# hangg7/soar

Hardware: AMD Instinct MI355X
Metric: fwd+bwd frames/sec @100k Gaussians, 1080p; achieved HBM GB/s vs roofline (higher is better)
Workload: dtype f32

## Files before the change

### include/soar_hip.h

```cpp
#ifndef SOAR_HIP_H
#define SOAR_HIP_H

#include <stddef.h>
#include <stdint.h>

#ifdef __cplusplus
extern "C" {
#endif

#define SOAR_HIP_ABI_VERSION 8

typedef struct SoarRastParams {
    int32_t P;
    int32_t W, H;
    int32_t sh_degree;
    int32_t M;
    int32_t prefiltered;
    int32_t render_front;
    int32_t sort_descending;
    int32_t debug;
    int32_t cfg_surface;
    int32_t cfg_normalize_depth;
    int32_t cfg_perpix_depth;
    int32_t cfg_lrn_cam;
// ... 234 lines not shown
                             SoarLossFinish *finish_out, void *stream);
int soar_frame_loss_pooled_partials(int32_t W, int32_t H, const float *color, const float *normal, const float *depth,
                                    const float *opac, const float *target_pool, int32_t n_sets, const int32_t *set_index_dev,
                                    float w_color, float w_mask, float w_normal, float w_depth, float *loss_out, float *scratch,
                                    float *dL_dcolor, float *dL_dnormal, float *dL_ddepth, float *dL_dopac, const void *image_buffer,
                                    const float *background, int32_t normalize_depth, SoarLossFinish *finish_out, void *stream);

#define SOAR_BACKWARD_LOSS_SCRATCH_FLOATS (4 * SOAR_FRAME_LOSS_SCRATCH_FLOATS)
typedef struct SoarBackwardLoss {
    const float *color, *normal, *depth, *opac;
    const float *target_color, *target_mask, *target_normal;
    const int32_t *set_index_dev;
    int32_t n_sets;
    float w_color, w_mask, w_normal, w_depth;
    float *loss_out;
    float *wave_sums;
} SoarBackwardLoss;
int soar_rast_backward_plan_loss(const SoarRastParams *prm, int32_t region,
                                 const float *means3D, const int32_t *radii, const float *shs,
                                 const float *colors_precomp, const float *scales, const float *rotations,
                                 const float *cov3D_precomp,
                                 const void *geom_buffer, const void *binning_buffer, const void *image_buffer,
                                 int64_t num_rendered, const SoarBackwardLoss *loss,
                                 float *dL_dmeans2D, float *dL_dcolors, float *dL_dopacity, float *dL_dmeans3D,
                                 float *dL_dcov3D, float *dL_dsh, float *dL_dscales, float *dL_drotations,
                                 float *dL_dviewmat, float *dL_dprojmat, float *dL_dcampos,
                                 void *workspace, size_t workspace_bytes, SoarLossFinish *finish_out,
                                 void *stream);
int soar_frames_geometry_warp_backward_wave_losses(int32_t n, const SoarFrameTail *frames, const float *xyz, const float *rot,
                                                   const float *weights, const float *joint_mats, int32_t P, int32_t J, const float *scales,
                                                   float *dL_dxyz, float *dL_drot, float *dL_dscales, float *dL_dcolors, float *dL_docc,
                                                   const SoarLossFinish *finish, void *stream);

typedef struct SoarAvatarLossArgs {
    int32_t H, W;
    float cos_limit, cos_weight;
    const float *render, *gt_rgb;
    const float *mask_img, *gt_mask;
    const float *normal, *gt_normal;
    const float *occ;
    const uint8_t *sel, *sel_normal, *sel_occ;
    float *stats, *stats_occ;
    float *scratch;
    const float *counts;
    const float *up_l1, *up_l1m, *up_cos, *up_occ, *up_ssim;
    const float *g_ssim;
    float *g_render, *g_mask, *g_normal, *g_occ;
    int32_t normal_raw;
    int32_t occ_grad_summed;
    float *cos_scale_out;
    const float *background;
} SoarAvatarLossArgs;
int soar_avatar_loss_scratch_floats(size_t *count);
int soar_avatar_pixel_losses(const SoarAvatarLossArgs *args, int32_t mode, void *stream);

int soar_ssim_scratch_floats(int32_t C, int32_t H, int32_t W, size_t *count);
int soar_ssim(int32_t C, int32_t H, int32_t W, const float *img1, const float *img2, float *ssim_out, float *scratch,
              float *dssim_dimg1, void *stream);
int soar_ssim_rendered(int32_t C, int32_t H, int32_t W, const float *img1, const float *img2, float *ssim_out, float *scratch,
                       float *dssim_dimg1, const float *rendered, void *stream);

typedef struct SoarDensifyRow {
    const float *src;
    float *dst;
    int32_t width;
    int32_t mode;
// ... 526 lines not shown
```

### soar_amd/csrc/lbs.hip

```cpp
#include "soar_common.h"
#include "loss_finish.h"
#include "geom_bwd_point.h"
#include "preprocess_point.h"
#include "soar_quat.h"

#pragma clang fp contract(on)

#ifndef SOAR_LBS_SKIP_UNUSED_JOINTS
#define SOAR_LBS_SKIP_UNUSED_JOINTS 1
#endif

namespace soar {

namespace {

constexpr int KNN_TILE = 1024;

__device__ __forceinline__ void quat_to_mat(const float q[4], float m[9])
{
    const float r = q[0], i = q[1], j = q[2], k = q[3];
    const float two_s = 2.0f / (r * r + i * i + j * j + k * k);
    m[0] = 1 - two_s * (j * j + k * k); m[1] = two_s * (i * j - k * r); m[2] = two_s * (i * k + j * r);
    m[3] = two_s * (i * j + k * r); m[4] = 1 - two_s * (i * i + k * k); m[5] = two_s * (j * k - i * r);
    m[6] = two_s * (i * k - j * r); m[7] = two_s * (j * k + i * r); m[8] = 1 - two_s * (i * i + j * j);
// ... 328 lines not shown
    }
#pragma unroll
    for (int h = 0; h < 2; h++) {
        const int o = tid + h * WARP_THREADS, c = o / WAVE, q = p0 + o % WAVE;
        if (o < 7 * WAVE && q < a.P) {
            if (c < 3) a.g_xyz[3 * q + c] = acc[h];
            else a.g_rot[4 * q + c - 3] = acc[h];
        }
    }
    if (p < a.P && k >= 1 && k - 1 < fs.n_extra) {
        const int e = k - 1, w = fs.width[e];
        const size_t count = (size_t)a.P * w;
        const float *src = fs.src[e] + (size_t)p * w;
        float *dst = fs.dst[e] + (size_t)p * w;
        for (int c0 = 0; c0 < w; c0 += 4) {
            float v[4][WARP_NF];
#pragma unroll
            for (int c = 0; c < 4; c++)
#pragma unroll
                for (int f = 0; f < WARP_NF; f++) v[c][f] = (c0 + c < w && f < n) ? src[(size_t)f * count + c0 + c] : 0.f;
#pragma unroll
            for (int c = 0; c < 4; c++) {
                if (c0 + c >= w) break;
                float s = v[c][0];
#pragma unroll
                for (int f = 1; f < WARP_NF; f++) s = f < n ? s + v[c][f] : s;
                for (int f = WARP_NF; f < n; f++) s += src[(size_t)f * count + c0 + c];
                dst[c0 + c] = s;
            }
        }
    }
}

__global__ void __launch_bounds__(WARP_THREADS) warp_preprocess_frames_kernel(WarpArgs a, int n, Batch<PreArgs> fr)
{
    extern __shared__ float wtile[];
    const int tid = threadIdx.x, k = __builtin_amdgcn_readfirstlane(tid / WAVE), lane = tid % WAVE;
    const int p0 = blockIdx.x * WAVE, p_raw = p0 + lane;
    stage_weight_rows(a, wtile, tid, p0);
    const int f = blockIdx.y * WARP_NF + k;
    if (f >= n) return;
    const bool in_range = p_raw < a.P;
    const int p = in_range ? p_raw : a.P - 1;
    float M[12], pos[3];
    float4 quat;
    blend_frame_matrix(wtile + (p - p0) * a.J, a.joint_mats + (size_t)f * a.mats_stride, a.J, M);
    forward_point_vals(a, p, M, pos, quat);
    float *xyz_out = a.xyz_out + (size_t)f * a.xyz_stride, *rot_out = a.rot_out + (size_t)f * a.rot_stride;
    xyz_out[3 * p] = pos[0]; xyz_out[3 * p + 1] = pos[1]; xyz_out[3 * p + 2] = pos[2];
    reinterpret_cast<float4 *>(rot_out)[p] = quat;
    const PreArgs &g = fr.v[f];
    PrePoint o;
    preprocess_point(g, p, in_range, pos[0], pos[1], pos[2], true, quat, o);
    preprocess_store(g, p, in_range, blockIdx.x, o);
    if (!g.prefiltered && blockIdx.x == 0 && lane == 0) g.header[H_PREFILTER_VIOLATIONS] = 0u;
}

constexpr int TAIL_C = 14;
struct TailOut {
    float *dL_dmeans2D[MAX_BATCH];
    float *dL_dscales, *dL_dcolors, *dL_docc;
};
struct TailLosses {
    int n, first_block;
    int per_wave;
    SoarLossFinish v[MAX_BATCH];
};
#ifndef SOAR_TAIL_WPE
#define SOAR_TAIL_WPE 4
#endif
__global__ void __launch_bounds__(WARP_THREADS) __attribute__((amdgpu_waves_per_eu(SOAR_TAIL_WPE, 8))) geom_warp_backward_frames_kernel(WarpArgs a, int n, Batch<GeomBwdArgs> fr, TailOut out, TailLosses losses)
{
    extern __shared__ __attribute__((aligned(16))) float wtile[];
    static_assert(WARP_THREADS == 256 && WARP_NF * TAIL_C * WAVE * sizeof(float) >= 256 * sizeof(float4), "loss_finish_sum: 256 threads, 4 KB of LDS");
    if (losses.n && (int)blockIdx.x >= losses.first_block) {
        const SoarLossFinish &l = losses.v[(int)blockIdx.x - losses.first_block];
        if (losses.per_wave) loss_finish_sum<true>(l.sums4, l.blocks, l.n, l.w_color, l.w_mask, l.w_normal, l.w_depth, l.loss_out, reinterpret_cast<float4 *>(wtile));
        else loss_finish_sum(l.sums4, l.blocks, l.n, l.w_color, l.w_mask, l.w_normal, l.w_depth, l.loss_out, reinterpret_cast<float4 *>(wtile));
        return;
    }
    float *red = wtile + WAVE * a.J;
    const int tid = threadIdx.x, k = __builtin_amdgcn_readfirstlane(tid / WAVE), lane = tid % WAVE;
    const int p0 = blockIdx.x * WAVE, p = p0 + lane;
    stage_weight_rows(a, wtile, tid, p0);
    constexpr int PER = (TAIL_C * WAVE + WARP_THREADS - 1) / WARP_THREADS;
    float acc[PER];
#pragma unroll
    for (int h = 0; h < PER; h++) acc[h] = 0.f;
    for (int f0 = 0; f0 < n; f0 += WARP_NF) {
        const int f = f0 + k;
        float d[TAIL_C];
#pragma unroll
        for (int c = 0; c < TAIL_C; c++) d[c] = 0.f;
        if (p < a.P && f < n) {
            const GeomBwdArgs &g = fr.v[f];
            GeomBwdPoint o;
            geometry_backward_point<false>(g, p, g.radii[p] > 0, o, nullptr, nullptr, nullptr);
            float *m2 = out.dL_dmeans2D[f];
            m2[3 * p + 0] = o.acc[0]; m2[3 * p + 1] = o.acc[1]; m2[3 * p + 2] = 0.f;
            float M[12], dx[3];
            float4 dq;
            blend_frame_matrix(wtile + lane * a.J, a.joint_mats + (size_t)f * a.mats_stride, a.J, M);
            backward_point_vals(a, p, M, o.g_mean[0], o.g_mean[1], o.g_mean[2], make_float4(o.g_rot[0], o.g_rot[1], o.g_rot[2], o.g_rot[3]), dx, dq);
            d[0] = dx[0]; d[1] = dx[1]; d[2] = dx[2]; d[3] = dq.x; d[4] = dq.y; d[5] = dq.z; d[6] = dq.w;
            d[7] = o.g_scale[0]; d[8] = o.g_scale[1]; d[9] = o.g_scale[2];
            d[10] = o.acc[6]; d[11] = o.acc[7]; d[12] = o.acc[8];
            d[13] = o.acc[13];
        }
        if (f0) __syncthreads();
#pragma unroll
        for (int c = 0; c < TAIL_C; c++) red[(k * TAIL_C + c) * WAVE + lane] = d[c];
        __syncthreads();
#pragma unroll
        for (int h = 0; h < PER; h++) {
            const int o = tid + h * WARP_THREADS;
            if (o < TAIL_C * WAVE)
#pragma unroll
                for (int kk = 0; kk < WARP_NF; kk++) acc[h] += red[kk * TAIL_C * WAVE + o];
        }
    }
#pragma unroll
    for (int h = 0; h < PER; h++) {
        const int o = tid + h * WARP_THREADS, c = o / WAVE, q = p0 + o % WAVE;
        if (o < TAIL_C * WAVE && q < a.P) {
            if (c < 3) a.g_xyz[3 * q + c] = acc[h];
            else if (c < 7) a.g_rot[4 * q + c - 3] = acc[h];
            else if (c < 10) out.dL_dscales[3 * q + c - 7] = acc[h];
            else if (c < 13) out.dL_dcolors[3 * q + c - 10] = acc[h];
            else if (out.dL_docc) out.dL_docc[q] = acc[h];
        }
    }
}

__global__ void __launch_bounds__(256) dist2_knn3_kernel(const float *__restrict__ pts, int N, float *__restrict__ out)
{
    __shared__ float tile[KNN_TILE * 3];
    const int tid = threadIdx.x;
    const int p = blockIdx.x * 256 + tid;
    const bool valid = p < N;
    float x = 0.f, y = 0.f, z = 0.f;
    if (valid) { x = pts[3 * p]; y = pts[3 * p + 1]; z = pts[3 * p + 2]; }
    float b0 = 3.402823466e+38f, b1 = b0, b2 = b0;
    for (int base = 0; base < N; base += KNN_TILE) {
        const int n = min(KNN_TILE, N - base);
        __syncthreads();
        for (int t = tid; t < n * 3; t += 256) tile[t] = pts[(size_t)base * 3 + t];
        __syncthreads();
        if (!valid) continue;
        for (int v = 0; v < n; v++) {
            const float ddx = x - tile[3 * v], ddy = y - tile[3 * v + 1], ddz = z - tile[3 * v + 2];
            float d = ddx * ddx + ddy * ddy + ddz * ddz;
            if (base + v == p) continue;
            if (d < b2) {
                b2 = d;
                if (b2 < b1) { const float t = b1; b1 = b2; b2 = t; }
                if (b1 < b0) { const float t = b0; b0 = b1; b1 = t; }
            }
        }
    }
    if (valid) out[p] = (b0 + b1 + b2) / 3.0f;
}

}

// ... 90 lines not shown

static int warp_backward_frames(const float *xyz, const float *rot, const float *weights, const float *joint_mats, const float *axis_perm,
                                size_t mats_stride, int32_t n, int32_t P, int32_t J, const float *dL_dxyz_out, const float *dL_drot_out,
                                float *dL_dxyz, float *dL_drot, int32_t n_extra, const float *const *extra_src, float *const *extra_dst,
                                const int32_t *extra_width, void *stream_)
{
    hipStream_t stream = static_cast<hipStream_t>(stream_);
    if (n <= 0 || !weights) { set_error("soar_lbs_warp_backward_sum: need n > 0 and blend weights"); return 1; }
    if (n_extra < 0 || n_extra > 2 || (n_extra > 0 && (!extra_src || !extra_dst || !extra_width))) {
        set_error("soar_lbs_warp_backward_sum: at most two extra blocks");
        return 1;
    }
    if (warp_check(xyz, rot, weights, joint_mats, P, J)) return 1;
    if (P == 0) return 0;
    if (!dL_dxyz_out || !dL_drot_out || !dL_dxyz || !dL_drot) { set_error("soar_lbs_warp_backward_sum: NULL pointer"); return 1; }
    WarpArgs a{};
    a.P = P; a.J = J; a.xyz = xyz; a.rot = rot; a.weights = weights; a.joint_mats = joint_mats;
    a.g_xyz_out = dL_dxyz_out; a.g_rot_out = dL_drot_out; a.g_xyz = dL_dxyz; a.g_rot = dL_drot;
    a.axis_perm = axis_perm;
    a.mats_stride = mats_stride; a.xyz_stride = (size_t)P * 3; a.rot_stride = (size_t)P * 4;
    FrameSums fs{};
    fs.n_extra = n_extra;
    for (int e = 0; e < n_extra; e++) {
        if (!extra_src[e] || !extra_dst[e] || extra_width[e] <= 0) { set_error("soar_lbs_warp_backward_sum: bad extra block %d", e); return 1; }
        fs.src[e] = extra_src[e]; fs.dst[e] = extra_dst[e]; fs.width[e] = extra_width[e];
    }
    const size_t lds = sizeof(float) * (WAVE * (size_t)J + WARP_NF * 7 * WAVE);
    StageTimer timer(ST_LBS_WARP_BWD, stream);
    hipLaunchKernelGGL(warp_backward_frames_kernel, dim3((P + WAVE - 1) / WAVE), dim3(WARP_THREADS), lds, stream, a, (int)n, fs);
    SOAR_LAUNCH_OK("lbs_warp_backward_sum", stream, 0);
    return 0;
}

int soar_frames_warp_preprocess(int32_t n, const SoarFrameHead *frames, const float *xyz, const float *rot, const float *weights,
                                const float *joint_mats, int32_t P, int32_t J, const float *colors, const float *opacities, const float *scales,
                                float *xyz_out, float *rot_out, void *stream_)
{
    hipStream_t stream = static_cast<hipStream_t>(stream_);
    const char *who = "soar_frames_warp_preprocess";
    if (n < 1 || n > MAX_BATCH || !frames) { set_error("%s: 1 <= n <= %d frames", who, MAX_BATCH); return 1; }
    if (!weights) { set_error("%s: needs the blend weights", who); return 1; }
    if (warp_check(xyz, rot, weights, joint_mats, P, J)) return 1;
    if (P == 0) return 0;
    if (!colors || !opacities || !scales || !xyz_out || !rot_out) { set_error("%s: a required pointer is NULL", who); return 1; }
    WarpArgs a{};
    a.P = P; a.J = J; a.xyz = xyz; a.rot = rot; a.weights = weights; a.joint_mats = joint_mats;
    a.xyz_out = xyz_out; a.rot_out = rot_out;
    a.mats_stride = (size_t)J * 16; a.xyz_stride = (size_t)P * 3; a.rot_stride = (size_t)P * 4;
    Batch<PreArgs> fr{};
    for (int f = 0; f < n; f++) {
        const SoarFrameHead &t = frames[f];
        if (!t.prm || !t.geom_buffer || !t.radii) { set_error("%s: frame %d: a pointer is NULL", who, f); return 1; }
        if (t.prm->P != P || t.prm->M != 0 || t.prm->prefiltered != 0) {
            set_error("%s: frame %d: needs P = %d Gaussians with explicit colours (M = 0), not prefiltered", who, f, P);
            return 1;
        }
        GeomBuf g;
        carve_geom(t.geom_buffer, P, 0, &g);
        fill_pre_args(fr.v[f], *t.prm, xyz_out + (size_t)f * a.xyz_stride, nullptr, colors, opacities, scales, rot_out + (size_t)f * a.rot_stride,
                      nullptr, g, t.radii);
    }
    const size_t lds = sizeof(float) * WAVE * (size_t)J;
    StageTimer timer(ST_LBS_WARP_FWD, stream);
    hipLaunchKernelGGL(warp_preprocess_frames_kernel, dim3((P + WAVE - 1) / WAVE, (n + WARP_NF - 1) / WARP_NF), dim3(WARP_THREADS), lds, stream,
                       a, (int)n, fr);
    SOAR_LAUNCH_OK("frames_warp_preprocess", stream, 0);
    return 0;
}

int soar_frames_geometry_warp_backward(int32_t n, const SoarFrameTail *frames, const float *xyz, const float *rot, const float *weights,
                                       const float *joint_mats, int32_t P, int32_t J, const float *scales, float *dL_dxyz, float *dL_drot,
                                       float *dL_dscales, float *dL_dcolors, float *dL_docc, void *stream_)
{
    return soar_frames_geometry_warp_backward_losses(n, frames, xyz, rot, weights, joint_mats, P, J, scales, dL_dxyz, dL_drot, dL_dscales,
                                                     dL_dcolors, dL_docc, nullptr, stream_);
}

static int frames_tail(int32_t n, const SoarFrameTail *frames, const float *xyz, const float *rot, const float *weights, const float *joint_mats,
                       int32_t P, int32_t J, const float *scales, float *dL_dxyz, float *dL_drot, float *dL_dscales, float *dL_dcolors,
                       float *dL_docc, const SoarLossFinish *finish, bool per_wave, const char *who, void *stream_);

int soar_frames_geometry_warp_backward_losses(int32_t n, const SoarFrameTail *frames, const float *xyz, const float *rot,
                                              const float *weights, const float *joint_mats, int32_t P, int32_t J, const float *scales,
                                              float *dL_dxyz, float *dL_drot, float *dL_dscales, float *dL_dcolors, float *dL_docc,
                                              const SoarLossFinish *finish, void *stream_)
{
    return frames_tail(n, frames, xyz, rot, weights, joint_mats, P, J, scales, dL_dxyz, dL_drot, dL_dscales, dL_dcolors, dL_docc, finish, false,
                       finish ? "soar_frames_geometry_warp_backward_losses" : "soar_frames_geometry_warp_backward", stream_);
}

int soar_frames_geometry_warp_backward_wave_losses(int32_t n, const SoarFrameTail *frames, const float *xyz, const float *rot,
                                                   const float *weights, const float *joint_mats, int32_t P, int32_t J, const float *scales,
                                                   float *dL_dxyz, float *dL_drot, float *dL_dscales, float *dL_dcolors, float *dL_docc,
                                                   const SoarLossFinish *finish, void *stream_)
{
    if (!finish) { set_error("soar_frames_geometry_warp_backward_wave_losses: finish is NULL"); return 1; }
    return frames_tail(n, frames, xyz, rot, weights, joint_mats, P, J, scales, dL_dxyz, dL_drot, dL_dscales, dL_dcolors, dL_docc, finish, true,
                       "soar_frames_geometry_warp_backward_wave_losses", stream_);
}

static int frames_tail(int32_t n, const SoarFrameTail *frames, const float *xyz, const float *rot, const float *weights, const float *joint_mats,
                       int32_t P, int32_t J, const float *scales, float *dL_dxyz, float *dL_drot, float *dL_dscales, float *dL_dcolors,
                       float *dL_docc, const SoarLossFinish *finish, bool per_wave, const char *who, void *stream_)
{
    hipStream_t stream = static_cast<hipStream_t>(stream_);
    if (n < 1 || n > MAX_BATCH || !frames) { set_error("%s: 1 <= n <= %d frames", who, MAX_BATCH); return 1; }
    if (!weights) { set_error("%s: needs the blend weights", who); return 1; }
    if (warp_check(xyz, rot, weights, joint_mats, P, J)) return 1;
    if (P == 0) return 0;
    if (!scales || !dL_dxyz || !dL_drot || !dL_dscales || !dL_dcolors) { set_error("%s: a required pointer is NULL", who); return 1; }
    WarpArgs a{};
    a.P = P; a.J = J; a.xyz = xyz; a.rot = rot; a.weights = weights; a.joint_mats = joint_mats;
    a.g_xyz = dL_dxyz; a.g_rot = dL_drot;
    a.mats_stride = (size_t)J * 16;
    Batch<GeomBwdArgs> fr{};
    TailOut out{};
    out.dL_dscales = dL_dscales; out.dL_dcolors = dL_dcolors; out.dL_docc = dL_docc;
    for (int f = 0; f < n; f++) {
        const SoarFrameTail &t = frames[f];
        if (!t.prm || !t.means3D || !t.rotations || !t.radii || !t.geom_buffer || !t.workspace || !t.dL_dmeans2D) {
            set_error("%s: frame %d: a pointer is NULL", who, f);
            return 1;
        }
        if (t.prm->P != P || t.prm->M != 0 || t.prm->cfg_lrn_cam != 0) {
            set_error("%s: frame %d: needs P = %d Gaussians with explicit colours (M = 0) and cfg_lrn_cam = 0", who, f, P);
            return 1;
        }
        GeomBuf g;
        carve_geom(const_cast<void *>(t.geom_buffer), P, 0, &g);
        fill_geom_bwd_args(fr.v[f], *t.prm, t.means3D, t.radii, nullptr, scales, t.rotations, nullptr, g, static_cast<const float *>(t.workspace));
        out.dL_dmeans2D[f] = t.dL_dmeans2D;
    }
    TailLosses losses{};
    const int blocks = (P + WAVE - 1) / WAVE;
    if (finish) {
        losses.n = n; losses.first_block = blocks; losses.per_wave = per_wave ? 1 : 0;
        for (int f = 0; f < n; f++) {
            const SoarLossFinish &l = finish[f];
            if (!l.sums4 || !l.loss_out || l.blocks < 1 || l.blocks > SOAR_FRAME_LOSS_SCRATCH_FLOATS / 4 || l.n < 1) {
                set_error("%s: frame %d: finish[] is not what %s left", who, f,
                          per_wave ? "soar_rast_backward_plan_loss" : "soar_frame_loss_partials");
                return 1;
            }
            losses.v[f] = l;
        }
    }
    const size_t lds = sizeof(float) * (WAVE * (size_t)J + WARP_NF * TAIL_C * WAVE);
    StageTimer timer(ST_LBS_WARP_BWD, stream);
    hipLaunchKernelGGL(geom_warp_backward_frames_kernel, dim3(blocks + losses.n), dim3(WARP_THREADS), lds, stream, a, (int)n, fr, out, losses);
    SOAR_LAUNCH_OK("frames_geometry_warp_backward", stream, 0);
    return 0;
}

int soar_dist2_knn3(const float *points, int32_t N, float *out, void *stream_)
{
    hipStream_t stream = static_cast<hipStream_t>(stream_);
    if (N < 0) { set_error("soar_dist2_knn3: N < 0"); return 1; }
    if (N == 0) return 0;
    if (!points || !out) { set_error("soar_dist2_knn3: NULL pointer"); return 1; }
    StageTimer timer(ST_DIST2, stream);
    hipLaunchKernelGGL(dist2_knn3_kernel, dim3((N + 255) / 256), dim3(256), 0, stream, points, N, out);
    SOAR_LAUNCH_OK("dist2_knn3", stream, 0);
    return 0;
}

}
```

### soar_amd/hip_lib.py

```python
from __future__ import annotations

import ctypes as C
import os
from typing import Optional

_HERE = os.path.dirname(os.path.abspath(__file__))
LIB_PATH = os.environ.get("SOAR_HIP_LIB") or os.path.join(_HERE, "_lib", "libsoar_hip.so")
if os.environ.get("SOAR_HIP_LIB"):
    import sys as _sys
    print(f"[soar_amd] SOAR_HIP_LIB is set: loading {LIB_PATH} instead of the in-tree build (development A/B runs only)", file=_sys.stderr)

FRAME_LOSS_SCRATCH_FLOATS = 4 * 2048
ABI_VERSION = 8
c_f32p = C.c_void_p
_vp = C.c_void_p


class SoarRastParams(C.Structure):
    _fields_ = [
        ("P", C.c_int32), ("W", C.c_int32), ("H", C.c_int32), ("sh_degree", C.c_int32), ("M", C.c_int32),
        ("prefiltered", C.c_int32), ("render_front", C.c_int32), ("sort_descending", C.c_int32), ("debug", C.c_int32),
        ("cfg_surface", C.c_int32), ("cfg_normalize_depth", C.c_int32), ("cfg_perpix_depth", C.c_int32),
        ("cfg_lrn_cam", C.c_int32),
        ("tanfovx", C.c_float), ("tanfovy", C.c_float), ("scale_modifier", C.c_float),
# ... 223 lines not shown
    "soar_rast_backward_plan": (C.c_int, [C.POINTER(SoarRastParams), C.c_int32] + [_vp] * 7 + [_vp, _vp, _vp, C.c_int64] + [_vp] * 4
                                + [_vp] * 11 + [_vp, C.c_size_t, _vp]),
    "soar_rast_backward_plan_loss": (C.c_int, [C.POINTER(SoarRastParams), C.c_int32] + [_vp] * 7 + [_vp, _vp, _vp, C.c_int64] + [_vp]
                                     + [_vp] * 11 + [_vp, C.c_size_t, _vp, _vp]),
    "soar_rast_backward_occ_plan": (C.c_int, [C.POINTER(SoarRastParams), C.c_int32] + [_vp] * 7 + [_vp, _vp, _vp, C.c_int64] + [_vp] * 6
                                    + [C.c_int32] + [_vp] * 12 + [_vp, C.c_size_t, _vp]),
    "soar_rast_backward_region_counts": (C.c_int, [C.POINTER(C.c_int64), C.POINTER(C.c_int64)]),
    "soar_batch_begin": (C.c_int, [C.c_int32]),
    "soar_batch_frame": (C.c_int, [C.c_int32]),
    "soar_batch_end": (C.c_int, []),
    "soar_rast_occ_backward": (C.c_int, [C.POINTER(SoarRastParams), _vp, _vp, _vp, C.c_int64, _vp, _vp, _vp]),
    "soar_rast_mark_visible": (C.c_int, [C.c_int32, _vp, _vp, _vp, _vp, _vp]),
    "soar_rast_export_state": (C.c_int, [C.POINTER(SoarRastParams), _vp, _vp, _vp, C.c_int64] + [_vp] * 17 + [_vp]),
    "soar_lbs_knn_weights_bytes": (C.c_int, [C.c_int32, C.c_int32, C.POINTER(C.c_size_t)]),
    "soar_lbs_knn_weights": (C.c_int, [_vp, C.c_int32, _vp, C.c_int32, _vp, C.c_int32, C.c_int32, _vp, _vp, _vp, C.c_size_t, _vp]),
    "soar_lbs_knn_grid_bytes": (C.c_int, [C.c_int32, C.POINTER(C.c_size_t)]),
    "soar_lbs_knn_query_bytes": (C.c_int, [C.c_int32, C.POINTER(C.c_size_t)]),
    "soar_lbs_knn_build_grid": (C.c_int, [_vp, C.c_int32, _vp, C.c_int32, _vp, _vp]),
    "soar_lbs_knn_query": (C.c_int, [_vp, C.c_int32, _vp, C.c_int32, _vp, C.c_int32, C.c_int32, _vp, _vp, _vp, C.c_size_t, _vp]),
    "soar_lbs_knn_query_ordered": (C.c_int, [_vp, C.c_int32, _vp, C.c_int32, _vp, C.c_int32, C.c_int32, _vp, C.c_int32, _vp, _vp,
                                             _vp, C.c_size_t, _vp]),
    "soar_lbs_knn_state_bytes": (C.c_int, [C.c_int32, C.POINTER(C.c_size_t)]),
    "soar_lbs_knn_query_state": (C.c_int, [_vp, C.c_int32, _vp, C.c_int32, _vp, C.c_int32, _vp, C.c_int32, _vp, _vp, _vp, C.c_size_t, _vp]),
    "soar_lbs_knn_refresh": (C.c_int, [_vp, C.c_int32, C.c_int32, _vp, C.c_int32, _vp, _vp, _vp, _vp, _vp]),
    "soar_lbs_warp_forward": (C.c_int, [_vp] * 6 + [C.c_int32, C.c_int32] + [_vp] * 4),
    "soar_lbs_warp_backward": (C.c_int, [_vp] * 5 + [C.c_int32, C.c_int32] + [_vp] * 5),
    "soar_lbs_warp_forward_batch": (C.c_int, [_vp] * 4 + [C.c_int32] * 3 + [_vp] * 3),
    "soar_lbs_warp_backward_sum": (C.c_int, [_vp] * 4 + [C.c_int32] * 3 + [_vp] * 4 + [C.c_int32, _vp, _vp, _vp, _vp]),
    "soar_frames_warp_preprocess": (C.c_int, [C.c_int32, _vp] + [_vp] * 4 + [C.c_int32, C.c_int32] + [_vp] * 6),
    "soar_rast_backward_rows": (C.c_int, [_vp] * 22),
    "soar_frames_geometry_warp_backward": (C.c_int, [C.c_int32, _vp] + [_vp] * 4 + [C.c_int32, C.c_int32] + [_vp] * 7),
    "soar_frames_geometry_warp_backward_losses": (C.c_int, [C.c_int32, _vp] + [_vp] * 4 + [C.c_int32, C.c_int32] + [_vp] * 8),
    "soar_frames_geometry_warp_backward_wave_losses": (C.c_int, [C.c_int32, _vp] + [_vp] * 4 + [C.c_int32, C.c_int32] + [_vp] * 8),
    "soar_dist2_knn3": (C.c_int, [_vp, C.c_int32, _vp, _vp]),
    "soar_depth2normal": (C.c_int, [C.c_int32, C.c_int32, _vp, _vp, C.c_float, C.c_float, C.c_float, C.c_float, _vp, _vp]),
    "soar_depth2normal_backward": (C.c_int, [C.c_int32, C.c_int32, _vp, _vp, C.c_float, C.c_float, C.c_float, C.c_float, _vp, _vp,
                                             _vp]),
    "soar_normal2curv": (C.c_int, [C.c_int32, C.c_int32, _vp, _vp, _vp, _vp]),
    "soar_normal2curv_backward": (C.c_int, [C.c_int32, C.c_int32, _vp, _vp, _vp, _vp, _vp]),
    "soar_view_finish": (C.c_int, [C.c_int32, C.c_int32, _vp, _vp, _vp, _vp, C.c_float, C.c_float, _vp, _vp, _vp, _vp]),
    "soar_view_finish_backward": (C.c_int, [C.c_int32, C.c_int32, _vp, _vp, _vp, _vp, C.c_float, C.c_float, _vp, _vp, _vp, _vp,
                                            _vp, _vp]),
    "soar_ssim_scratch_floats": (C.c_int, [C.c_int32, C.c_int32, C.c_int32, C.POINTER(C.c_size_t)]),
    "soar_ssim": (C.c_int, [C.c_int32, C.c_int32, C.c_int32, _vp, _vp, _vp, _vp, _vp, _vp]),
    "soar_ssim_rendered": (C.c_int, [C.c_int32, C.c_int32, C.c_int32, _vp, _vp, _vp, _vp, _vp, _vp, _vp]),
    "soar_densify_stats": (C.c_int, [C.c_int32, _vp, _vp, C.c_int32, _vp, _vp, _vp, _vp, _vp, _vp]),
    "soar_densify_plan_bytes": (C.c_int, [C.c_int32, C.POINTER(C.c_size_t)]),
    "soar_densify_plan": (C.c_int, [C.c_int32, _vp, _vp, _vp, C.c_int32, C.c_int32, C.c_float, C.c_float, C.c_float, C.c_float,
                                    C.c_float, _vp, C.POINTER(C.c_int64), _vp]),
    "soar_densify_flags": (C.c_int, [C.c_int32, _vp, _vp, _vp]),
    "soar_densify_apply": (C.c_int, [C.c_int32, C.c_int32, _vp, C.c_int32, C.POINTER(SoarDensifyRow), _vp, _vp, _vp, C.c_int32, _vp]),
    "soar_smplx_joint_mats": (C.c_int, [C.c_int32, C.c_int32, C.c_int32, _vp, C.c_int32, _vp, _vp, _vp, _vp, _vp, _vp, _vp, _vp]),
    "soar_image_loss_scratch_floats": (C.c_int, [C.POINTER(C.c_size_t)]),
    "soar_masked_l1": (C.c_int, [C.c_int32, C.c_int32, C.c_int32, _vp, _vp, _vp, _vp, _vp, _vp]),
    "soar_masked_l1_backward": (C.c_int, [C.c_int32, C.c_int32, C.c_int32, _vp, _vp, _vp, _vp, _vp, _vp, _vp]),
    "soar_cos_loss": (C.c_int, [C.c_int32, C.c_int32, C.c_int32, _vp, _vp, _vp, C.c_float, C.c_float, _vp, _vp, _vp]),
    "soar_cos_loss_backward": (C.c_int, [C.c_int32, C.c_int32, C.c_int32, _vp, _vp, _vp, C.c_float, C.c_float, _vp, _vp, _vp, _vp]),
    "soar_frame_loss": (C.c_int, [C.c_int32, C.c_int32, _vp, _vp, _vp, _vp, _vp, _vp, _vp, C.c_float, C.c_float, C.c_float,
                                  C.c_float, _vp, _vp, _vp, _vp, _vp, _vp, _vp, _vp, C.c_int32, _vp]),
    "soar_frame_loss_pooled": (C.c_int, [C.c_int32, C.c_int32, _vp, _vp, _vp, _vp, _vp, C.c_int32, _vp, C.c_float, C.c_float, C.c_float,
                                         C.c_float, _vp, _vp, _vp, _vp, _vp, _vp, _vp, _vp, C.c_int32, _vp]),
    "soar_frame_loss_partials": (C.c_int, [C.c_int32, C.c_int32, _vp, _vp, _vp, _vp, _vp, _vp, _vp, C.c_float, C.c_float, C.c_float,
                                           C.c_float, _vp, _vp, _vp, _vp, _vp, _vp, _vp, _vp, C.c_int32, _vp, _vp]),
    "soar_frame_loss_pooled_partials": (C.c_int, [C.c_int32, C.c_int32, _vp, _vp, _vp, _vp, _vp, C.c_int32, _vp, C.c_float, C.c_float,
                                                  C.c_float, C.c_float, _vp, _vp, _vp, _vp, _vp, _vp, _vp, _vp, C.c_int32, _vp, _vp]),
    "soar_selftest_exp": (C.c_int, [_vp, C.c_int32, _vp, _vp, _vp]),
# ... 165 lines not shown
```

### soar_amd/step_plan.py

```python
from __future__ import annotations

import ctypes as C
import os
from typing import Dict, List, Optional, Sequence

import torch

from . import hip_lib
from .hip_lib import check, ptr
from .rasterizer import _Ctx


class FrameStepPlan:
    def __init__(self, seq, n_frames: int, targets: Dict[str, torch.Tensor], bg: torch.Tensor, capacity: int, flat,
                 loss_weights: Sequence[float] = (1.0, 1.0, 0.1, 0.01), use_graphs: bool = True, batched: Optional[bool] = None,
                 loss: str = "synthetic", lambdas: Optional[Dict[str, float]] = None):
        if loss not in ("synthetic", "avatar"):
            raise ValueError(f"loss must be 'synthetic' or 'avatar', got {loss!r}")
        self.loss_kind = loss
        if loss == "avatar" and (use_graphs or not torch.is_tensor(targets)):
            raise ValueError("loss='avatar' needs a resident target pool and use_graphs=False")
        L = hip_lib.lib()
        self.L, self.seq, self.flat, self.n = L, seq, flat, int(n_frames)
        dev = seq.device
# ... 32 lines not shown
        for i in range(self.n):
            v = dict(
                xyz_p=self.xyz_p_all[i], rot_p=self.rot_p_all[i], radii=torch.empty((P,), dtype=torch.int32, device=dev),
                color=torch.empty((3, H, W), **f), normal=torch.empty((3, H, W), **f), depth=torch.empty((1, H, W), **f),
                opac=torch.empty((1, H, W), **f), occ=torch.empty((3, H, W), **f),
                geom=torch.empty(geom_b, **u8), img=torch.empty(img_b, **u8), binning=torch.empty(bin_b, **u8),
                work=torch.empty(work_b, **u8), loss=torch.empty((), **f), sums=torch.empty((hip_lib.FRAME_LOSS_SCRATCH_FLOATS,), **f),
                gC=torch.empty((3, H, W), **f), gN=torch.empty((3, H, W), **f), gD=torch.empty((1, H, W), **f),
                gO=torch.empty((1, H, W), **f),
                g_means2D=torch.empty((P, 3), **f), g_colors=torch.empty((P, 3), **f), g_opacity=torch.empty((P, 1), **f),
                g_means3D=self.g_means3D_all[i], g_cov3D=torch.empty((P, 6), **f), g_scales=torch.empty((P, 3), **f),
                g_rot_p=self.g_rot_p_all[i], g_view=torch.empty((4, 4), **f), g_proj=torch.empty((4, 4), **f),
                g_campos=torch.empty((3,), **f))
            v["geom"][:256].zero_()
            self.views.append(v)
        self.fused_tail = os.environ.get("SOAR_PLAN_FUSED_TAIL", "1") != "0" and self.n <= 8
        if self.fused_tail:
            self.ctx.params.debug |= 8
            self._tail_frames = (hip_lib.SoarFrameTail * self.n)()
            for i, v in enumerate(self.views):
                t = self._tail_frames[i]
                t.prm = C.addressof(self.ctx.params)
                t.means3D, t.rotations, t.radii = v["xyz_p"].data_ptr(), v["rot_p"].data_ptr(), v["radii"].data_ptr()
                t.geom_buffer, t.workspace, t.dL_dmeans2D = v["geom"].data_ptr(), v["work"].data_ptr(), v["g_means2D"].data_ptr()
        env = os.environ.get("SOAR_PLAN_BWD_REGION")
        self.bwd_region = int(env) if env in ("1", "2") else (2 if W * H >= (1 << 20) else 1)
        self.fused_head = os.environ.get("SOAR_PLAN_FUSED_HEAD", "1") != "0" and self.n <= 8
        if self.fused_head:
            self.ctx.params.debug |= 16
            self._head_frames = (hip_lib.SoarFrameHead * self.n)()
            for i, v in enumerate(self.views):
                h = self._head_frames[i]
                h.prm, h.geom_buffer, h.radii = C.addressof(self.ctx.params), v["geom"].data_ptr(), v["radii"].data_ptr()
        self.g_xyz = torch.empty((self.n, P, 3), **f)
        self.g_rot = torch.empty((self.n, P, 4), **f)
        self.g_scales = torch.empty((self.n, P, 3), **f)
        self.g_colors = torch.empty((self.n, P, 3), **f)
        self.losses = torch.empty((self.n,), **f)
        from . import lbs as _lbs
        self.knn = _lbs.KnnFollower(seq.knn_grid, P)
        for name in ("opacity", "occ"):
            if name in flat.views:
                flat.views[name].zero_()
        if loss == "avatar":
            self._setup_avatar(lambdas)
        self.steps = 0
        self.STAMP_CAP = 8192
        self.stamps = torch.zeros((1 + 2 * self.STAMP_CAP,), dtype=torch.int64, device=dev) if os.environ.get("SOAR_PLAN_TIMESTAMPS") in ("1", "2") else None
        self.fine_stamps = os.environ.get("SOAR_PLAN_TIMESTAMPS") == "2"
        self.stale = None
        self._baked = self._leaf_signature()
        self.streams = [torch.cuda.Stream(device=dev) for _ in range(self.n)]
        if batched is None:
            env = os.environ.get("SOAR_PLAN_BATCHED")
            batched = (env != "0") if env in ("0", "1") else (self.W * self.H <= 3_000_000)
        self.batched = bool(batched) and self.n <= 8
        fold = self.batched and not use_graphs
        self.loss_in_tail = fold and self.fused_tail and loss == "synthetic" and os.environ.get("SOAR_PLAN_LOSS_IN_TAIL", "1") != "0"
        if self.loss_in_tail:
            self._loss_finish = (hip_lib.SoarLossFinish * self.n)()
        self.loss_in_backward = self.loss_in_tail and os.environ.get("SOAR_PLAN_LOSS_IN_BACKWARD", "1") != "0"
        if self.loss_in_backward:
            self._loss_records = (hip_lib.SoarBackwardLoss * self.n)()
            for v in self.views:
                v["wave_sums"] = torch.empty((hip_lib.BACKWARD_LOSS_SCRATCH_FLOATS,), **f)
        self.gather_in_adam = fold and self.n <= 8 and os.environ.get("SOAR_PLAN_GATHER_IN_ADAM", "1") != "0"
# ... 115 lines not shown
    def _stage_stamp(self, i: int, stage: int, stream: int) -> None:
        if self.stamps is not None and self.fine_stamps:
            self._stamp(100 + 10 * i + stage, stream)

    def _gather_args(self):
        s = self.seq
        n_sets = int(self.pool.shape[0]) if self.pool is not None else 0
        return (self.n, s.num_frames, 55 * 16, n_sets, (C.c_int32 * self.n)(*self._frames_now), ptr(s.cano2live), ptr(self.mats), ptr(self.frame_sel))

    def _prologue(self, stream: int, resort: bool = True, gathered: bool = False) -> None:
        L, s = self.L, self.seq
        self._stamp(0, stream)
        n_sets = int(self.pool.shape[0]) if self.pool is not None else 0
        if gathered:
            pass
        elif self._ids_by_value:
            ids = (C.c_int32 * self.n)(*self._frames_now)
            check(L.soar_gather_step_inputs_ids(self.n, s.num_frames, 55 * 16, n_sets, ids, ptr(s.cano2live), ptr(self.mats),
                                                ptr(self.frame_sel), stream), "gather_step_inputs")
        else:
            check(L.soar_gather_step_inputs(self.n, s.num_frames, 55 * 16, n_sets, ptr(self.frame_ids), ptr(s.cano2live), ptr(self.mats),
                                            ptr(self.frame_sel), stream), "gather_step_inputs")
        if resort:
            self.knn.full(s.xyz.detach(), self.blend_weights, stream)
        else:
            self.knn.calls = 1
            self.knn.refresh(s.xyz.detach(), self.blend_weights, stream)
        self._stamp(1, stream)

    def _warp_all(self, stream: int) -> None:
        L, s = self.L, self.seq
        J = int(self.blend_weights.shape[1])
        if self.fused_head:
            check(L.soar_frames_warp_preprocess(self.n, self._head_frames, ptr(s.xyz.detach()), ptr(s.rot.detach()), ptr(self.blend_weights),
                                                ptr(self.mats), self.P, J, ptr(s.colors.detach()), ptr(self.ones), ptr(s.scales.detach()),
                                                ptr(self.xyz_p_all), ptr(self.rot_p_all), stream), "frames_warp_preprocess")
            return
        check(L.soar_lbs_warp_forward_batch(ptr(s.xyz.detach()), ptr(s.rot.detach()), ptr(self.blend_weights), ptr(self.mats), self.n,
                                            self.P, J, ptr(self.xyz_p_all), ptr(self.rot_p_all), stream), "warp_forward_batch")

    def _call(self, key, build) -> None:
        c = self._call_cache.get(key)
        if c is None:
            c = self._call_cache[key] = build()
        if c[0](*c[1]) != 0:
            check(1, c[2])

    def _f_geometry(self, i: int, stream: int) -> None:
        def build():
            L, s, v = self.L, self.seq, self.views[i]
            return (L.soar_rast_forward_geometry, (C.byref(self.ctx.params), ptr(v["xyz_p"]), None, ptr(s.colors.detach()), ptr(self.ones),
                                                   ptr(s.scales.detach()), ptr(v["rot_p"]), None, ptr(v["geom"]), ptr(v["radii"]), None, stream),
                    "geometry")
        self._call(("geometry", i, stream), build)

    def _f_render(self, i: int, stream: int) -> None:
        def build():
            L, s, v = self.L, self.seq, self.views[i]
            return (L.soar_rast_forward_render_occ, (C.byref(self.ctx.params), ptr(v["radii"]), ptr(v["geom"]), ptr(v["binning"]), ptr(v["img"]),
                                                     self.capacity, ptr(v["color"]), ptr(v["normal"]), ptr(v["depth"]), ptr(v["opac"]),
                                                     ptr(s.occ), ptr(v["occ"]), stream), "render")
        self._call(("render", i, stream), build)

    def _f_loss(self, i: int, stream: int) -> None:
        def build():
            L, v, W, H = self.L, self.views[i], self.W, self.H
# ... 95 lines not shown
            try:
                for stage in stages:
                    for k, i in enumerate(frames):
                        check(L.soar_batch_frame(k), "batch_frame")
                        stage(i, stream)
            finally:
                L.soar_batch_end()
        if self.loss_kind == "avatar":
            from .losses import _AvatarStageLoss as S
            batch((self._f_geometry, self._f_render, self._av_finish, self._av_ssim, self._av_pixel, self._f_backward_occ))
            if len(frames) == self.n:
                torch.addmv(self.av_occ_terms_all[:, 0] * self.av_occ_up[0], self.av_terms_all, self.av_coef, out=self.losses)
            else:
                for i in frames:
                    v = self.views[i]
                    torch.add(torch.dot(v["terms"], self.av_coef), v["occ_terms"][0] * self.av_occ_up[0], out=self.losses[i])
        elif self.loss_in_backward:
            batch((self._f_geometry, self._f_render, self._f_backward_loss))
        else:
            batch((self._f_geometry, self._f_render, self._f_loss, self._f_backward))
        for i in frames:
            self._stamp(3 + 2 * i, stream)

    def _epilogue(self, stream: int) -> None:
        L, s = self.L, self.seq
        self._stamp(2 * self.n + 2, stream)
        J = int(self.blend_weights.shape[1])
        fv = self.flat.views
        src = (C.c_void_p * 2)(ptr(self.g_scales), ptr(self.g_colors))
        dst = (C.c_void_p * 2)(ptr(fv["scales"]), ptr(fv["colors"]))
        width = (C.c_int32 * 2)(3, 3)
        if self.fused_tail:
            occ = ptr(fv["occ"]) if (self.loss_kind == "avatar" and "occ" in fv) else None
            if self.loss_in_tail:
                tail = L.soar_frames_geometry_warp_backward_wave_losses if self.loss_in_backward else L.soar_frames_geometry_warp_backward_losses
                check(tail(self.n, self._tail_frames, ptr(s.xyz.detach()), ptr(s.rot.detach()),
                                                                  ptr(self.blend_weights), ptr(self.mats), self.P, J, ptr(s.scales.detach()),
                                                                  ptr(fv["xyz"]), ptr(fv["rot"]), ptr(fv["scales"]), ptr(fv["colors"]), occ,
                                                                  self._loss_finish, stream), "frames_geometry_warp_backward_losses")
            else:
                check(L.soar_frames_geometry_warp_backward(self.n, self._tail_frames, ptr(s.xyz.detach()), ptr(s.rot.detach()), ptr(self.blend_weights),
                                                           ptr(self.mats), self.P, J, ptr(s.scales.detach()), ptr(fv["xyz"]), ptr(fv["rot"]),
                                                           ptr(fv["scales"]), ptr(fv["colors"]), occ, stream), "frames_geometry_warp_backward")
            self._stamp(2 * self.n + 3, stream)
            return
        check(L.soar_lbs_warp_backward_sum(ptr(s.xyz.detach()), ptr(s.rot.detach()), ptr(self.blend_weights), ptr(self.mats), self.n,
                                           self.P, J, ptr(self.g_means3D_all), ptr(self.g_rot_p_all), ptr(fv["xyz"]), ptr(fv["rot"]),
                                           2, src, dst, width, stream), "warp_backward_sum")
        if self.loss_kind == "avatar" and "occ" in fv:
            check(L.soar_sum_frames(self.n, self.P, ptr(self.g_occ_all), ptr(fv["occ"]), stream), "sum_frames")
        self._stamp(2 * self.n + 3, stream)

    def _capture(self) -> None:
        dev = self.device
        self.frame_ids.copy_(torch.arange(self.n, dtype=torch.int32) % max(self.seq.num_frames, 1))
        self._run_eager()
        torch.cuda.synchronize(dev)
        cap = torch.cuda.Stream(device=dev)
        graphs = {}
        with torch.cuda.device(dev):
            for name, resort in (("prologue_resort", True), ("prologue", False)):
                g = torch.cuda.CUDAGraph()
                with torch.cuda.graph(g, stream=cap):
                    self._prologue(cap.cuda_stream, resort)
                graphs[name] = g
                g = torch.cuda.CUDAGraph()
                with torch.cuda.graph(g, stream=cap):
# ... 104 lines not shown
```

Baseline: 5827.

## Hand over blended per-point skinning matrices from forward warp to backward tail

The forward warp/preprocess kernel now writes each point's blended 3x4 skinning matrix to a planar per-frame buffer. The fused backward tail kernel reads it back instead of restaging blend-weight rows into LDS and re-blending joint matrices. This removes the J-wide weight reads and blend arithmetic from the backward pass and frees LDS. In exchange it adds 48 bytes per point per frame of HBM writes and reads, plus a persistent buffer. The change also adds new entry points and lowers the tail kernel's waves-per-EU hint.

```diff
diff --git a/include/soar_hip.h b/include/soar_hip.h
--- a/include/soar_hip.h
+++ b/include/soar_hip.h
@@ -290,6 +290,17 @@
                                                    float *dL_dxyz, float *dL_drot, float *dL_dscales, float *dL_dcolors, float *dL_docc,
                                                    const SoarLossFinish *finish, void *stream);
 
+int soar_frames_warp_preprocess_mats(int32_t n, const SoarFrameHead *frames, const float *xyz, const float *rot, const float *weights,
+                                     const float *joint_mats, int32_t P, int32_t J, const float *colors, const float *opacities,
+                                     const float *scales, float *xyz_out, float *rot_out, float *mats_out, void *stream);
+int soar_frames_geometry_warp_backward_mats_losses(int32_t n, const SoarFrameTail *frames, const float *xyz, const float *rot, const float *mats,
+                                                   int32_t P, const float *scales, float *dL_dxyz, float *dL_drot, float *dL_dscales,
+                                                   float *dL_dcolors, float *dL_docc, const SoarLossFinish *finish, void *stream);
+int soar_frames_geometry_warp_backward_mats_wave_losses(int32_t n, const SoarFrameTail *frames, const float *xyz, const float *rot,
+                                                        const float *mats, int32_t P, const float *scales, float *dL_dxyz, float *dL_drot,
+                                                        float *dL_dscales, float *dL_dcolors, float *dL_docc, const SoarLossFinish *finish,
+                                                        void *stream);
+
 typedef struct SoarAvatarLossArgs {
     int32_t H, W;
     float cos_limit, cos_weight;
diff --git a/soar_amd/csrc/lbs.hip b/soar_amd/csrc/lbs.hip
--- a/soar_amd/csrc/lbs.hip
+++ b/soar_amd/csrc/lbs.hip
@@ -384,7 +384,38 @@
     }
 }
 
-__global__ void __launch_bounds__(WARP_THREADS) warp_preprocess_frames_kernel(WarpArgs a, int n, Batch<PreArgs> fr)
+#ifndef SOAR_HANDOVER_PLANES
+#define SOAR_HANDOVER_PLANES 1
+#endif
+__device__ __forceinline__ void handover_store(float *mats, int f, int p, int P, const float M[12])
+{
+#if SOAR_HANDOVER_PLANES
+    float *o = mats + (size_t)f * 12 * P + p;
+#pragma unroll
+    for (int c = 0; c < 12; c++) o[(size_t)c * P] = M[c];
+#else
+    float4 *o = reinterpret_cast<float4 *>(mats + ((size_t)f * P + p) * 12);
+    o[0] = make_float4(M[0], M[1], M[2], M[3]);
+    o[1] = make_float4(M[4], M[5], M[6], M[7]);
+    o[2] = make_float4(M[8], M[9], M[10], M[11]);
+#endif
+}
+__device__ __forceinline__ void handover_load(const float *mats, int f, int p, int P, float M[12])
+{
+#if SOAR_HANDOVER_PLANES
+    const float *m = mats + (size_t)f * 12 * P + p;
+#pragma unroll
+    for (int c = 0; c < 12; c++) M[c] = m[(size_t)c * P];
+#else
+    const float4 *m = reinterpret_cast<const float4 *>(mats + ((size_t)f * P + p) * 12);
+    const float4 r0 = m[0], r1 = m[1], r2 = m[2];
+    M[0] = r0.x; M[1] = r0.y; M[2] = r0.z; M[3] = r0.w;
+    M[4] = r1.x; M[5] = r1.y; M[6] = r1.z; M[7] = r1.w;
+    M[8] = r2.x; M[9] = r2.y; M[10] = r2.z; M[11] = r2.w;
+#endif
+}
+template <bool HANDOVER>
+__device__ __forceinline__ void warp_preprocess_frames_body(const WarpArgs &a, int n, const Batch<PreArgs> &fr, float *mats_out)
 {
     extern __shared__ float wtile[];
     const int tid = threadIdx.x, k = __builtin_amdgcn_readfirstlane(tid / WAVE), lane = tid % WAVE;
@@ -397,6 +428,7 @@
     float M[12], pos[3];
     float4 quat;
     blend_frame_matrix(wtile + (p - p0) * a.J, a.joint_mats + (size_t)f * a.mats_stride, a.J, M);
+    if (HANDOVER) handover_store(mats_out, f, p, a.P, M);
     forward_point_vals(a, p, M, pos, quat);
     float *xyz_out = a.xyz_out + (size_t)f * a.xyz_stride, *rot_out = a.rot_out + (size_t)f * a.rot_stride;
     xyz_out[3 * p] = pos[0]; xyz_out[3 * p + 1] = pos[1]; xyz_out[3 * p + 2] = pos[2];
@@ -406,6 +438,14 @@
     preprocess_point(g, p, in_range, pos[0], pos[1], pos[2], true, quat, o);
     preprocess_store(g, p, in_range, blockIdx.x, o);
     if (!g.prefiltered && blockIdx.x == 0 && lane == 0) g.header[H_PREFILTER_VIOLATIONS] = 0u;
+}
+__global__ void __launch_bounds__(WARP_THREADS) warp_preprocess_frames_kernel(WarpArgs a, int n, Batch<PreArgs> fr)
+{
+    warp_preprocess_frames_body<false>(a, n, fr, nullptr);
+}
+__global__ void __launch_bounds__(WARP_THREADS) warp_preprocess_frames_handover_kernel(WarpArgs a, int n, Batch<PreArgs> fr, float *mats_out)
+{
+    warp_preprocess_frames_body<true>(a, n, fr, mats_out);
 }
 
 constexpr int TAIL_C = 14;
@@ -421,7 +461,12 @@
 #ifndef SOAR_TAIL_WPE
 #define SOAR_TAIL_WPE 4
 #endif
-__global__ void __launch_bounds__(WARP_THREADS) __attribute__((amdgpu_waves_per_eu(SOAR_TAIL_WPE, 8))) geom_warp_backward_frames_kernel(WarpArgs a, int n, Batch<GeomBwdArgs> fr, TailOut out, TailLosses losses)
+#ifndef SOAR_TAIL_HANDOVER_EARLY
+#define SOAR_TAIL_HANDOVER_EARLY 1
+#endif
+template <bool HANDOVER>
+__device__ __forceinline__ void geom_warp_backward_frames_body(const WarpArgs &a, int n, const Batch<GeomBwdArgs> &fr, const TailOut &out,
+                                                               const TailLosses &losses, const float *__restrict__ mats_in)
 {
     extern __shared__ __attribute__((aligned(16))) float wtile[];
     static_assert(WARP_THREADS == 256 && WARP_NF * TAIL_C * WAVE * sizeof(float) >= 256 * sizeof(float4), "loss_finish_sum: 256 threads, 4 KB of LDS");
@@ -431,10 +476,10 @@
         else loss_finish_sum(l.sums4, l.blocks, l.n, l.w_color, l.w_mask, l.w_normal, l.w_depth, l.loss_out, reinterpret_cast<float4 *>(wtile));
         return;
     }
-    float *red = wtile + WAVE * a.J;
+    float *red = HANDOVER ? wtile : wtile + WAVE * a.J;
     const int tid = threadIdx.x, k = __builtin_amdgcn_readfirstlane(tid / WAVE), lane = tid % WAVE;
     const int p0 = blockIdx.x * WAVE, p = p0 + lane;
-    stage_weight_rows(a, wtile, tid, p0);
+    if (!HANDOVER) stage_weight_rows(a, wtile, tid, p0);
     constexpr int PER = (TAIL_C * WAVE + WARP_THREADS - 1) / WARP_THREADS;
     float acc[PER];
 #pragma unroll
@@ -447,12 +492,14 @@
         if (p < a.P && f < n) {
             const GeomBwdArgs &g = fr.v[f];
             GeomBwdPoint o;
+            float M[12], dx[3];
+            if (HANDOVER && SOAR_TAIL_HANDOVER_EARLY) handover_load(mats_in, f, p, a.P, M);
             geometry_backward_point<false>(g, p, g.radii[p] > 0, o, nullptr, nullptr, nullptr);
             float *m2 = out.dL_dmeans2D[f];
             m2[3 * p + 0] = o.acc[0]; m2[3 * p + 1] = o.acc[1]; m2[3 * p + 2] = 0.f;
-            float M[12], dx[3];
             float4 dq;
-            blend_frame_matrix(wtile + lane * a.J, a.joint_mats + (size_t)f * a.mats_stride, a.J, M);
+            if (HANDOVER && !SOAR_TAIL_HANDOVER_EARLY) handover_load(mats_in, f, p, a.P, M);
+            if (!HANDOVER) blend_frame_matrix(wtile + lane * a.J, a.joint_mats + (size_t)f * a.mats_stride, a.J, M);
             backward_point_vals(a, p, M, o.g_mean[0], o.g_mean[1], o.g_mean[2], make_float4(o.g_rot[0], o.g_rot[1], o.g_rot[2], o.g_rot[3]), dx, dq);
             d[0] = dx[0]; d[1] = dx[1]; d[2] = dx[2]; d[3] = dq.x; d[4] = dq.y; d[5] = dq.z; d[6] = dq.w;
             d[7] = o.g_scale[0]; d[8] = o.g_scale[1]; d[9] = o.g_scale[2];
@@ -482,6 +529,17 @@
             else if (out.dL_docc) out.dL_docc[q] = acc[h];
         }
     }
+}
+__global__ void __launch_bounds__(WARP_THREADS) __attribute__((amdgpu_waves_per_eu(SOAR_TAIL_WPE, 8))) geom_warp_backward_frames_kernel(WarpArgs a, int n, Batch<GeomBwdArgs> fr, TailOut out, TailLosses losses)
+{
+    geom_warp_backward_frames_body<false>(a, n, fr, out, losses, nullptr);
+}
+#ifndef SOAR_TAIL_HANDOVER_WPE
+#define SOAR_TAIL_HANDOVER_WPE 3
+#endif
+__global__ void __launch_bounds__(WARP_THREADS) __attribute__((amdgpu_waves_per_eu(SOAR_TAIL_HANDOVER_WPE, 8))) geom_warp_backward_frames_handover_kernel(WarpArgs a, int n, Batch<GeomBwdArgs> fr, TailOut out, TailLosses losses, const float *__restrict__ mats_in)
+{
+    geom_warp_backward_frames_body<true>(a, n, fr, out, losses, mats_in);
 }
 
 __global__ void __launch_bounds__(256) dist2_knn3_kernel(const float *__restrict__ pts, int N, float *__restrict__ out)
@@ -638,12 +696,32 @@
     return 0;
 }
 
+static int frames_head(int32_t n, const SoarFrameHead *frames, const float *xyz, const float *rot, const float *weights,
+                       const float *joint_mats, int32_t P, int32_t J, const float *colors, const float *opacities, const float *scales,
+                       float *xyz_out, float *rot_out, float *mats_out, const char *who, void *stream_);
+
 int soar_frames_warp_preprocess(int32_t n, const SoarFrameHead *frames, const float *xyz, const float *rot, const float *weights,
                                 const float *joint_mats, int32_t P, int32_t J, const float *colors, const float *opacities, const float *scales,
                                 float *xyz_out, float *rot_out, void *stream_)
 {
+    return frames_head(n, frames, xyz, rot, weights, joint_mats, P, J, colors, opacities, scales, xyz_out, rot_out, nullptr,
+                       "soar_frames_warp_preprocess", stream_);
+}
+
+int soar_frames_warp_preprocess_mats(int32_t n, const SoarFrameHead *frames, const float *xyz, const float *rot, const float *weights,
+                                     const float *joint_mats, int32_t P, int32_t J, const float *colors, const float *opacities,
+                                     const float *scales, float *xyz_out, float *rot_out, float *mats_out, void *stream_)
+{
+    const char *who = "soar_frames_warp_preprocess_mats";
+    if (!mats_out || (reinterpret_cast<uintptr_t>(mats_out) & 15)) { set_error("%s: mats_out is NULL or not 16-byte aligned", who); return 1; }
+    return frames_head(n, frames, xyz, rot, weights, joint_mats, P, J, colors, opacities, scales, xyz_out, rot_out, mats_out, who, stream_);
+}
+
+static int frames_head(int32_t n, const SoarFrameHead *frames, const float *xyz, const float *rot, const float *weights,
+                       const float *joint_mats, int32_t P, int32_t J, const float *colors, const float *opacities, const float *scales,
+                       float *xyz_out, float *rot_out, float *mats_out, const char *who, void *stream_)
+{
     hipStream_t stream = static_cast<hipStream_t>(stream_);
-    const char *who = "soar_frames_warp_preprocess";
     if (n < 1 || n > MAX_BATCH || !frames) { set_error("%s: 1 <= n <= %d frames", who, MAX_BATCH); return 1; }
     if (!weights) { set_error("%s: needs the blend weights", who); return 1; }
     if (warp_check(xyz, rot, weights, joint_mats, P, J)) return 1;
@@ -668,8 +746,9 @@
     }
     const size_t lds = sizeof(float) * WAVE * (size_t)J;
     StageTimer timer(ST_LBS_WARP_FWD, stream);
-    hipLaunchKernelGGL(warp_preprocess_frames_kernel, dim3((P + WAVE - 1) / WAVE, (n + WARP_NF - 1) / WARP_NF), dim3(WARP_THREADS), lds, stream,
-                       a, (int)n, fr);
+    const dim3 grid((P + WAVE - 1) / WAVE, (n + WARP_NF - 1) / WARP_NF);
+    if (mats_out) hipLaunchKernelGGL(warp_preprocess_frames_handover_kernel, grid, dim3(WARP_THREADS), lds, stream, a, (int)n, fr, mats_out);
+    else hipLaunchKernelGGL(warp_preprocess_frames_kernel, grid, dim3(WARP_THREADS), lds, stream, a, (int)n, fr);
     SOAR_LAUNCH_OK("frames_warp_preprocess", stream, 0);
     return 0;
 }
@@ -684,7 +763,7 @@
 
 static int frames_tail(int32_t n, const SoarFrameTail *frames, const float *xyz, const float *rot, const float *weights, const float *joint_mats,
                        int32_t P, int32_t J, const float *scales, float *dL_dxyz, float *dL_drot, float *dL_dscales, float *dL_dcolors,
-                       float *dL_docc, const SoarLossFinish *finish, bool per_wave, const char *who, void *stream_);
+                       float *dL_docc, const SoarLossFinish *finish, bool per_wave, const char *who, void *stream_, const float *mats_in = nullptr);
 
 int soar_frames_geometry_warp_backward_losses(int32_t n, const SoarFrameTail *frames, const float *xyz, const float *rot,
                                               const float *weights, const float *joint_mats, int32_t P, int32_t J, const float *scales,
@@ -705,14 +784,40 @@
                        "soar_frames_geometry_warp_backward_wave_losses", stream_);
 }
 
+int soar_frames_geometry_warp_backward_mats_losses(int32_t n, const SoarFrameTail *frames, const float *xyz, const float *rot, const float *mats,
+                                                   int32_t P, const float *scales, float *dL_dxyz, float *dL_drot, float *dL_dscales,
+                                                   float *dL_dcolors, float *dL_docc, const SoarLossFinish *finish, void *stream_)
+{
+    const char *who = "soar_frames_geometry_warp_backward_mats_losses";
+    if (!mats || (reinterpret_cast<uintptr_t>(mats) & 15)) { set_error("%s: mats is NULL or not 16-byte aligned", who); return 1; }
+    return frames_tail(n, frames, xyz, rot, nullptr, nullptr, P, 0, scales, dL_dxyz, dL_drot, dL_dscales, dL_dcolors, dL_docc, finish, false, who,
+                       stream_, mats);
+}
+
+int soar_frames_geometry_warp_backward_mats_wave_losses(int32_t n, const SoarFrameTail *frames, const float *xyz, const float *rot,
+                                                        const float *mats, int32_t P, const float *scales, float *dL_dxyz, float *dL_drot,
+                                                        float *dL_dscales, float *dL_dcolors, float *dL_docc, const SoarLossFinish *finish,
+                                                        void *stream_)
+{
+    const char *who = "soar_frames_geometry_warp_backward_mats_wave_losses";
+    if (!finish) { set_error("%s: finish is NULL", who); return 1; }
+    if (!mats || (reinterpret_cast<uintptr_t>(mats) & 15)) { set_error("%s: mats is NULL or not 16-byte aligned", who); return 1; }
+    return frames_tail(n, frames, xyz, rot, nullptr, nullptr, P, 0, scales, dL_dxyz, dL_drot, dL_dscales, dL_dcolors, dL_docc, finish, true, who,
+                       stream_, mats);
+}
+
 static int frames_tail(int32_t n, const SoarFrameTail *frames, const float *xyz, const float *rot, const float *weights, const float *joint_mats,
                        int32_t P, int32_t J, const float *scales, float *dL_dxyz, float *dL_drot, float *dL_dscales, float *dL_dcolors,
-                       float *dL_docc, const SoarLossFinish *finish, bool per_wave, const char *who, void *stream_)
+                       float *dL_docc, const SoarLossFinish *finish, bool per_wave, const char *who, void *stream_, const float *mats_in)
 {
     hipStream_t stream = static_cast<hipStream_t>(stream_);
     if (n < 1 || n > MAX_BATCH || !frames) { set_error("%s: 1 <= n <= %d frames", who, MAX_BATCH); return 1; }
-    if (!weights) { set_error("%s: needs the blend weights", who); return 1; }
-    if (warp_check(xyz, rot, weights, joint_mats, P, J)) return 1;
+    if (mats_in) {
+        if (P < 0 || (P > 0 && (!xyz || !rot))) { set_error("%s: bad P = %d or a NULL pointer", who, P); return 1; }
+    } else {
+        if (!weights) { set_error("%s: needs the blend weights", who); return 1; }
+        if (warp_check(xyz, rot, weights, joint_mats, P, J)) return 1;
+    }
     if (P == 0) return 0;
     if (!scales || !dL_dxyz || !dL_drot || !dL_dscales || !dL_dcolors) { set_error("%s: a required pointer is NULL", who); return 1; }
     WarpArgs a{};
@@ -751,9 +856,13 @@
             losses.v[f] = l;
         }
     }
-    const size_t lds = sizeof(float) * (WAVE * (size_t)J + WARP_NF * TAIL_C * WAVE);
+    const size_t lds = sizeof(float) * ((mats_in ? 0 : WAVE * (size_t)J) + WARP_NF * TAIL_C * WAVE);
     StageTimer timer(ST_LBS_WARP_BWD, stream);
-    hipLaunchKernelGGL(geom_warp_backward_frames_kernel, dim3(blocks + losses.n), dim3(WARP_THREADS), lds, stream, a, (int)n, fr, out, losses);
+    if (mats_in)
+        hipLaunchKernelGGL(geom_warp_backward_frames_handover_kernel, dim3(blocks + losses.n), dim3(WARP_THREADS), lds, stream, a, (int)n, fr, out,
+                           losses, mats_in);
+    else
+        hipLaunchKernelGGL(geom_warp_backward_frames_kernel, dim3(blocks + losses.n), dim3(WARP_THREADS), lds, stream, a, (int)n, fr, out, losses);
     SOAR_LAUNCH_OK("frames_geometry_warp_backward", stream, 0);
     return 0;
 }
diff --git a/soar_amd/hip_lib.py b/soar_amd/hip_lib.py
--- a/soar_amd/hip_lib.py
+++ b/soar_amd/hip_lib.py
@@ -279,6 +279,9 @@
     "soar_frames_geometry_warp_backward": (C.c_int, [C.c_int32, _vp] + [_vp] * 4 + [C.c_int32, C.c_int32] + [_vp] * 7),
     "soar_frames_geometry_warp_backward_losses": (C.c_int, [C.c_int32, _vp] + [_vp] * 4 + [C.c_int32, C.c_int32] + [_vp] * 8),
     "soar_frames_geometry_warp_backward_wave_losses": (C.c_int, [C.c_int32, _vp] + [_vp] * 4 + [C.c_int32, C.c_int32] + [_vp] * 8),
+    "soar_frames_warp_preprocess_mats": (C.c_int, [C.c_int32, _vp] + [_vp] * 4 + [C.c_int32, C.c_int32] + [_vp] * 7),
+    "soar_frames_geometry_warp_backward_mats_losses": (C.c_int, [C.c_int32, _vp] + [_vp] * 3 + [C.c_int32] + [_vp] * 8),
+    "soar_frames_geometry_warp_backward_mats_wave_losses": (C.c_int, [C.c_int32, _vp] + [_vp] * 3 + [C.c_int32] + [_vp] * 8),
     "soar_dist2_knn3": (C.c_int, [_vp, C.c_int32, _vp, _vp]),
     "soar_depth2normal": (C.c_int, [C.c_int32, C.c_int32, _vp, _vp, C.c_float, C.c_float, C.c_float, C.c_float, _vp, _vp]),
     "soar_depth2normal_backward": (C.c_int, [C.c_int32, C.c_int32, _vp, _vp, C.c_float, C.c_float, C.c_float, C.c_float, _vp, _vp,
diff --git a/soar_amd/step_plan.py b/soar_amd/step_plan.py
--- a/soar_amd/step_plan.py
+++ b/soar_amd/step_plan.py
@@ -88,6 +88,9 @@
             for i, v in enumerate(self.views):
                 h = self._head_frames[i]
                 h.prm, h.geom_buffer, h.radii = C.addressof(self.ctx.params), v["geom"].data_ptr(), v["radii"].data_ptr()
+        self.blend_handover = self.fused_head and self.fused_tail and os.environ.get("SOAR_PLAN_BLEND_HANDOVER", "1") != "0"
+        if self.blend_handover:
+            self.pt_mats = torch.empty((self.n, 12, P), **f)
         self.g_xyz = torch.empty((self.n, P, 3), **f)
         self.g_rot = torch.empty((self.n, P, 4), **f)
         self.g_scales = torch.empty((self.n, P, 3), **f)
@@ -269,6 +272,12 @@
         L, s = self.L, self.seq
         J = int(self.blend_weights.shape[1])
         if self.fused_head:
+            if self.blend_handover:
+                check(L.soar_frames_warp_preprocess_mats(self.n, self._head_frames, ptr(s.xyz.detach()), ptr(s.rot.detach()), ptr(self.blend_weights),
+                                                         ptr(self.mats), self.P, J, ptr(s.colors.detach()), ptr(self.ones), ptr(s.scales.detach()),
+                                                         ptr(self.xyz_p_all), ptr(self.rot_p_all), ptr(self.pt_mats), stream),
+                      "frames_warp_preprocess_mats")
+                return
             check(L.soar_frames_warp_preprocess(self.n, self._head_frames, ptr(s.xyz.detach()), ptr(s.rot.detach()), ptr(self.blend_weights),
                                                 ptr(self.mats), self.P, J, ptr(s.colors.detach()), ptr(self.ones), ptr(s.scales.detach()),
                                                 ptr(self.xyz_p_all), ptr(self.rot_p_all), stream), "frames_warp_preprocess")
@@ -430,7 +439,12 @@
         width = (C.c_int32 * 2)(3, 3)
         if self.fused_tail:
             occ = ptr(fv["occ"]) if (self.loss_kind == "avatar" and "occ" in fv) else None
-            if self.loss_in_tail:
+            if self.blend_handover:
+                tail = L.soar_frames_geometry_warp_backward_mats_wave_losses if self.loss_in_backward else L.soar_frames_geometry_warp_backward_mats_losses
+                check(tail(self.n, self._tail_frames, ptr(s.xyz.detach()), ptr(s.rot.detach()), ptr(self.pt_mats), self.P, ptr(s.scales.detach()),
+                           ptr(fv["xyz"]), ptr(fv["rot"]), ptr(fv["scales"]), ptr(fv["colors"]), occ,
+                           self._loss_finish if self.loss_in_tail else None, stream), "frames_geometry_warp_backward_mats_losses")
+            elif self.loss_in_tail:
                 tail = L.soar_frames_geometry_warp_backward_wave_losses if self.loss_in_backward else L.soar_frames_geometry_warp_backward_losses
                 check(tail(self.n, self._tail_frames, ptr(s.xyz.detach()), ptr(s.rot.detach()),
                                                                   ptr(self.blend_weights), ptr(self.mats), self.P, J, ptr(s.scales.detach()),
```

Result: no change. 5872, median of 6 (+0.8%).
